# XinkeAE/Active-ORB-SLAM2

Hardware: AMD Instinct MI355X
Metric: frames/sec (extract+match+localBA) TUM 640x480 (higher is better)
Workload: dtype u8 (extract, match) + f64 (PoseOptimization, LocalBA)

## Files before the change

active-orb-slam2_amd/capi.py:

```python
from __future__ import annotations

import ctypes as C
import os

import numpy as np

_HERE = os.path.dirname(os.path.abspath(__file__))
_LIB = None

AOS2_OK = 0
AOS2_ERR_ARG, AOS2_ERR_CAPACITY, AOS2_ERR_TOO_SMALL, AOS2_ERR_HIP, AOS2_ERR_NO_DEVICE = -1, -2, -3, -4, -5
AOS2_ERR_STOPPED = 1

KP_DTYPE = np.dtype([("x", "<f4"), ("y", "<f4"), ("size", "<f4"), ("angle", "<f4"),
                     ("response", "<f4"), ("octave", "<i4"), ("class_id", "<i4")])


class LibraryMissing(RuntimeError):
    pass


class AosError(RuntimeError):
    def __init__(self, code, msg):
        super().__init__(f"aos2 error {code}: {msg}")
# ... 23 lines not shown
        for n in ("scale_factors", "inv_scale_factors", "sigma2", "inv_sigma2"):
            f = getattr(L, "aos2_extractor_" + n)
            f.argtypes = [vp]
            f.restype = C.POINTER(cf)
        for n in ("features_per_level", "umax"):
            f = getattr(L, "aos2_extractor_" + n)
            f.argtypes = [vp]
            f.restype = C.POINTER(ci)
        L.aos2_extractor_max_keypoints.argtypes = [vp]
        L.aos2_extractor_max_keypoints_for.argtypes = [vp, ci, ci]
        L.aos2_extractor_extract.argtypes = [vp, vp, ci, ci, ci, vp, vp, ci, C.POINTER(ci)]
        L.aos2_extractor_extract_batch.argtypes = [vp, vp, ci, ci, ci, ci, C.c_size_t, vp, vp, ci, vp]
        L.aos2_host_alloc.argtypes = [C.POINTER(vp), C.c_size_t]
        L.aos2_host_free.argtypes = [vp]
        L.aos2_extractor_extract_batch_device.argtypes = [vp, vp, ci, ci, ci, ci, C.c_size_t, vp, vp, ci, vp]
        L.aos2_extractor_extract_batch_device_async.argtypes = [vp, vp, ci, ci, ci, ci, C.c_size_t, vp, vp, ci, vp]
        L.aos2_extractor_wait.argtypes = [vp]
        L.aos2_extractor_pyramid_level_size.argtypes = [vp, ci, C.POINTER(ci), C.POINTER(ci)]
        L.aos2_extractor_pyramid_level.argtypes = [vp, ci, ci, ci, vp, ci]
        L.aos2_extractor_debug_candidates.argtypes = [vp, ci, ci, vp, vp, vp, ci, C.POINTER(ci)]
        L.aos2_extractor_last_timing.argtypes = [vp, vp, ci]
        if hasattr(L, "aos2_extractor_set_chunks"):
            L.aos2_extractor_set_chunks.argtypes = [vp, ci]
        L.aos2_extractor_bench_fast.argtypes = [vp, ci, C.POINTER(cf)]
        L.aos2_extractor_bench_describe.argtypes = [vp, ci, C.POINTER(cf)]
        if hasattr(L, "aos2_compute_stereo_matches"):
            L.aos2_compute_stereo_matches.argtypes = [vp, vp, ci, vp, vp, ci, vp, vp, ci, cf, cf, vp, vp]
            L.aos2_compute_stereo_matches_device.argtypes = [vp, vp, ci, vp, vp, vp, vp, vp, vp, ci, cf, cf, vp, vp]
            L.aos2_compute_stereo_matches_device_async.argtypes = [vp, vp, ci, vp, vp, vp, vp, vp, vp, ci, cf, cf, vp, vp]
            L.aos2_compute_stereo_matches_last_device_ms.restype = cf
            L.aos2_compute_stereo_matches_last_device_ms.argtypes = [vp]
        if hasattr(L, "aos2_vocabulary_create"):
            L.aos2_vocabulary_create.argtypes = [ci, C.POINTER(vp)]
            L.aos2_vocabulary_destroy.argtypes = [vp]
            L.aos2_vocabulary_load_binary.argtypes = [vp, C.c_char_p]
            L.aos2_vocabulary_load_text.argtypes = [vp, C.c_char_p]
            L.aos2_vocabulary_save_binary.argtypes = [vp, C.c_char_p]
            L.aos2_vocabulary_set_nodes.argtypes = [vp, ci, ci, ci, ci, ci, vp, vp, vp, vp]
            for nm in ("k", "levels", "scoring", "weighting", "nodes", "empty"):
                getattr(L, "aos2_vocabulary_" + nm).argtypes = [vp]
            L.aos2_vocabulary_size.argtypes = [vp]
            L.aos2_vocabulary_get_nodes.argtypes = [vp] * 6
            L.aos2_vocabulary_size.restype = C.c_uint
            L.aos2_vocabulary_transform.argtypes = [vp, vp, ci, ci, vp, vp, C.POINTER(ci), vp, vp, vp, C.POINTER(ci), vp, vp]
            L.aos2_vocabulary_transform_device.argtypes = [vp, ci, vp, vp, ci, ci] + [vp] * 9
            L.aos2_vocabulary_last_device_ms.restype = cf
            L.aos2_vocabulary_last_device_ms.argtypes = [vp]
            L.aos2_vocabulary_score.argtypes = [vp, vp, vp, ci, vp, vp, ci, C.POINTER(C.c_double)]
        L.aos2_debug_octree_host.argtypes = [vp, vp, vp, ci, ci, ci, ci, ci, ci, vp, ci]
        L.aos2_debug_sincos_host.argtypes = [cf, C.POINTER(cf), C.POINTER(cf)]
        L.aos2_debug_extractor_plan.argtypes = [vp, ci, ci, vp, vp, ci, C.POINTER(ci), vp]
        L.aos2_debug_sincos_device.argtypes = [vp, ci, vp, vp, ci]
        L.aos2_debug_wave_ops_device.argtypes = [vp, vp, ci, ci, vp, vp, ci]
        L.aos2_debug_pose_blocks_device.argtypes = [vp, vp, vp, vp, vp, vp, vp, ci, ci]
        L.aos2_debug_lba_reduced_solve_device.argtypes = [ci] + [vp] * 12 + [ci]
        L.aos2_debug_triangulate_host.argtypes = [vp, ci, vp, vp, vp, vp]
        L.aos2_triangulate_matches.argtypes = [vp, vp, ci, vp, vp, vp, vp]
        L.aos2_debug_sim3_host.argtypes = [vp, vp, ci]
        L.aos2_sim3_ransac.argtypes = [vp, vp, vp, ci]
        L.aos2_debug_pnp_host.argtypes = [vp, vp, ci]
        L.aos2_debug_pnp_set.argtypes = [ci, vp, ci, vp]
        L.aos2_debug_pnp_scan.argtypes = [ci, ci, vp, vp, ci, ci, ci, vp, vp, vp]
        L.aos2_pnp_ransac.argtypes = [vp, vp, vp, ci]
        L.aos2_pnp_ransac_parameters.argtypes = [ci, C.c_double, ci, ci, ci, cf, vp, vp, vp]
        L.aos2_debug_sim3_opt_host.argtypes = [vp, vp, ci]
        L.aos2_optimize_sim3.argtypes = [vp, vp, vp, ci]
        L.aos2_optimize_sim3_last_device_ms.argtypes = [vp]
        L.aos2_optimize_sim3_last_device_ms.restype = cf
        if hasattr(L, "aos2_matcher_create"):
            L.aos2_matcher_create.argtypes = [cf, ci, ci, C.POINTER(vp)]
            L.aos2_matcher_destroy.argtypes = [vp]
            L.aos2_descriptor_distance.argtypes = [vp, vp]
            if hasattr(L, "aos2_matcher_last_device_ms"):
                L.aos2_matcher_last_device_ms.argtypes = [vp]
                L.aos2_matcher_last_device_ms.restype = cf
            L.aos2_matcher_hamming_best2.argtypes = [vp, vp, ci, vp, ci, vp, vp, vp]
            L.aos2_matcher_hamming_best2_device.argtypes = [vp, vp, ci, vp, ci, vp, vp, vp, ci, C.POINTER(cf)]
            L.aos2_matcher_search_by_bow.argtypes = [vp, vp, ci, vp, vp]
            L.aos2_matcher_search_by_bow_device.argtypes = [vp, vp, ci, vp, vp]
            L.aos2_matcher_search_by_bow_frames.argtypes = [vp, vp, vp, vp]
            L.aos2_vocabulary_stream.argtypes = [vp]
            L.aos2_vocabulary_stream.restype = vp
            if hasattr(L, "aos2_matcher_search_by_bow_kf"):
                L.aos2_matcher_search_by_bow_kf.argtypes = [vp, vp, ci, vp, vp]
                L.aos2_matcher_search_for_triangulation.argtypes = [vp, vp, ci, ci, vp, vp]
                L.aos2_compute_distinctive_descriptors.argtypes = [vp, ci, vp, vp, vp]
            if hasattr(L, "aos2_matcher_fuse"):
                L.aos2_matcher_fuse.argtypes = [vp, vp, vp, ci, vp, vp, vp]
                L.aos2_matcher_search_by_projection_kf.argtypes = [vp, vp, vp, vp, vp]
                L.aos2_matcher_search_by_sim3.argtypes = [vp, vp, vp, vp, vp, vp, vp]
                L.aos2_matcher_search_by_projection_reloc.argtypes = [vp, vp, vp, ci, vp, vp]
            if hasattr(L, "aos2_frame_assign_features_to_grid"):
                L.aos2_frame_assign_features_to_grid.argtypes = [vp, ci, vp, vp, cf, cf, cf, cf, vp, vp, C.POINTER(C.c_int32)]
                L.aos2_frame_stereo_from_rgbd.argtypes = [vp, ci, vp, vp, vp, vp, ci, ci, ci, cf, vp, vp]
            if hasattr(L, "aos2_frame_is_in_frustum"):
                L.aos2_frame_is_in_frustum.argtypes = [vp, vp, cf, cf, cf, cf, ci, cf, vp, vp, vp, vp, vp, vp]
            if hasattr(L, "aos2_matcher_search_for_initialization"):
                L.aos2_matcher_search_for_initialization.argtypes = [vp, vp, ci, vp, vp, vp, vp, ci, vp, vp]
            if hasattr(L, "aos2_matcher_search_by_projection_batch"):
                L.aos2_matcher_search_by_projection_batch.argtypes = [vp, vp, vp, ci, cf, vp, vp]
            L.aos2_matcher_search_by_projection.argtypes = [vp, vp, vp, cf, vp, vp]
            L.aos2_matcher_search_by_projection_last.argtypes = [vp, vp, vp, cf, ci, vp, vp]
        if hasattr(L, "aos2_lba_create"):
            L.aos2_lba_create.argtypes = [ci, C.POINTER(vp)]
            L.aos2_lba_destroy.argtypes = [vp]
            L.aos2_lba_solve.argtypes = [vp, vp, vp]
# ... 833 lines not shown
        for k, a in zip(names, arr):
            setattr(P[i], k, a.ctypes.data)
        for tag, K in (("1", q["K1"]), ("2", q["K2"])):
            for name, v in zip(("fx", "fy", "cx", "cy"), K):
                setattr(P[i], name + tag, float(np.float32(v)))
        P[i].q12 = (C.c_double * 4)(*[float(v) for v in q["q12"]])
        P[i].t12 = (C.c_double * 3)(*[float(v) for v in q["t12"]])
        P[i].s12, P[i].th2, P[i].fix_scale = float(q["s12"]), float(np.float32(q["th2"])), int(bool(q["fix_scale"]))
        R[i].outlier = out.ctypes.data
        if sentinel is not None:
            C.memset(C.byref(R[i]), sentinel, _Sim3OptResult.outlier.offset)
            R[i].n_bad = R[i].n_inliers = sentinel
    return P, R, keep, outs


def _sim3_opt_results(R, outs):
    return [dict(q12=np.array(R[i].q12, np.float64), t12=np.array(R[i].t12, np.float64), s12=np.float64(R[i].s12), outlier=out,
                 n_bad=R[i].n_bad, n_inliers=R[i].n_inliers, iterations=tuple(R[i].iterations), trials=tuple(R[i].trials))
            for i, out in enumerate(outs)]


def debug_sim3_opt_host(problems):
    P, R, keep, outs = _sim3_opt_args(problems)
    _check(lib().aos2_debug_sim3_opt_host(P, R, len(problems)))
    return _sim3_opt_results(R, outs)


def debug_sincos_device(angles, device=0):
    a = np.ascontiguousarray(angles, np.float32)
    s = np.zeros_like(a)
    c = np.zeros_like(a)
    _check(lib().aos2_debug_sincos_device(_p(a), len(a), _p(s), _p(c), device))
    return s, c


WAVE_OPS_I = ("dpp_u32_B1", "dpp_u32_4E", "dpp_u32_141", "dpp_u32_140", "dpp_i32_B1", "dpp_i32_4E", "dpp_i32_141", "dpp_i32_140",
              "row_sum", "sum", "max", "row_min", "min", "incl_scan", "block_excl_scan", "block_total")
WAVE_OPS_D = ("dpp_f64_B1", "dpp_f64_4E", "dpp_f64_141", "dpp_f64_140", "row_sum_f64", "readlane_0", "readlane_63")


def debug_wave_ops_device(vi, vd, device=0):
    vi = np.ascontiguousarray(vi, np.int32); vd = np.ascontiguousarray(vd, np.float64)
    assert vi.ndim == 2 and vi.shape == vd.shape
    oi = np.zeros(vi.shape + (len(WAVE_OPS_I),), np.int32)
    od = np.zeros(vi.shape + (len(WAVE_OPS_D),), np.float64)
    _check(lib().aos2_debug_wave_ops_device(_p(vi), _p(vd), vi.shape[0], vi.shape[1], _p(oi), _p(od), device))
    out = {k: oi[..., j].copy() for j, k in enumerate(WAVE_OPS_I)}
    out.update({k: od[..., j].copy() for j, k in enumerate(WAVE_OPS_D)})
    for k in ("row_min", "min"):
        out[k] = out[k].view(np.uint32)
    return out


def debug_pose_blocks_device(upd, T, Hb, lam, x0, device=0):
    upd = np.ascontiguousarray(upd, np.float64); T = np.ascontiguousarray(T, np.float64)
    Hb = np.ascontiguousarray(Hb, np.float64); lam = np.ascontiguousarray(lam, np.float64)
    x = np.ascontiguousarray(x0, np.float64).copy()
    n = len(lam)
    To = np.zeros((n, 7)); ok = np.zeros(n, np.uint8)
    _check(lib().aos2_debug_pose_blocks_device(_p(upd), _p(T), _p(To), _p(Hb), _p(lam), _p(x), _p(ok), n, device))
    return To, x, ok


def debug_lba_reduced_solve_device(cases, device=0):
    cat = lambda k, dt=np.float64: np.ascontiguousarray(np.concatenate([np.asarray(c[k], dt).ravel() for c in cases]))
    nps = np.array([np.asarray(c["bs"]).size // 6 for c in cases], np.int32)
    for c, q in zip(cases, nps):
        assert np.asarray(c["H"]).shape == (6 * q, 6 * q) and np.asarray(c["T"]).shape == (q, 7)
        assert all(np.asarray(c[k]).shape == (6 * q,) for k in ("bs", "b_pose", "x0", "scale0"))
    form = np.array([c["form"] for c in cases], np.int32)
    H, bs, bp, T, x, sc = cat("H"), cat("bs"), cat("b_pose"), cat("T"), cat("x0"), cat("scale0")
    lam = np.array([c["lam"] for c in cases], np.float64)
    To, Tb, ok = np.zeros_like(T), np.zeros_like(T), np.zeros(len(cases), np.uint8)
    _check(lib().aos2_debug_lba_reduced_solve_device(len(cases), _p(nps), _p(form), _p(H), _p(bs), _p(bp), _p(lam), _p(T), _p(x), _p(To), _p(Tb),
                                                     _p(sc), _p(ok), device))
    out, o6, o7 = [], 0, 0
    for q, k in zip(nps, ok):
        out.append(dict(ok=int(k), x=x[o6:o6 + 6 * q].copy(), scale_terms=sc[o6:o6 + 6 * q].copy(),
                        T_out=To[o7:o7 + 7 * q].reshape(q, 7).copy(), T_backup=Tb[o7:o7 + 7 * q].reshape(q, 7).copy()))
        o6 += 6 * q; o7 += 7 * q
    return out


class _BowPair(C.Structure):
    _fields_ = [("n_kf", C.c_int32), ("n_f", C.c_int32), ("desc_kf", C.c_void_p), ("desc_f", C.c_void_p),
                ("kf_has_mp", C.c_void_p), ("angle_kf", C.c_void_p), ("angle_f", C.c_void_p),
                ("n_nodes_kf", C.c_int32), ("n_nodes_f", C.c_int32),
                ("node_id_kf", C.c_void_p), ("node_off_kf", C.c_void_p), ("node_idx_kf", C.c_void_p),
                ("node_id_f", C.c_void_p), ("node_off_f", C.c_void_p), ("node_idx_f", C.c_void_p)]


class _BowFrames(C.Structure):
    _fields_ = [("n_frames", C.c_int32), ("cap", C.c_int32)] + [(k, C.c_void_p) for k in (
        "d_desc_kf", "d_kps_kf", "d_n_kf", "d_desc_f", "d_kps_f", "d_n_f", "kf_has_mp", "d_kf_fv_node", "d_kf_fv_off", "d_kf_fv_idx",
        "d_kf_n_fv", "d_f_fv_node", "d_f_fv_off", "d_f_fv_idx", "d_f_n_fv")]


class _BowKfPair(C.Structure):
    _fields_ = [("n1", C.c_int32), ("n2", C.c_int32), ("desc1", C.c_void_p), ("desc2", C.c_void_p),
                ("has_mp1", C.c_void_p), ("has_mp2", C.c_void_p), ("angle1", C.c_void_p), ("angle2", C.c_void_p),
                ("n_nodes1", C.c_int32), ("n_nodes2", C.c_int32),
                ("node_id1", C.c_void_p), ("node_off1", C.c_void_p), ("node_idx1", C.c_void_p),
                ("node_id2", C.c_void_p), ("node_off2", C.c_void_p), ("node_idx2", C.c_void_p)]


class _TriangPair(C.Structure):
# ... 663 lines not shown
```

active-orb-slam2_amd/csrc/debug_taps.hip:

```cpp
#include <algorithm>
#include <cmath>
#include <vector>

#include "aos2_common.h"
#include "octree.h"
#include "pnp.h"
#include "sincos_exact.h"
#include "sim3.h"
#include "triangulate.h"
#include "wave_ops.h"

namespace aos2 {
__global__ void sincos_kernel(const float *a, int n, float *s, float *c)
{
    const int i = blockIdx.x * blockDim.x + threadIdx.x;
    if (i < n) sincos_exact(a[i], &s[i], &c[i]);
}

constexpr int kWaveOpsI = 16, kWaveOpsD = 7;
template <int NT>
__global__ __launch_bounds__(NT) void wave_ops_kernel(const int32_t *vi, const double *vd, int32_t *out_i, double *out_d)
{
    __shared__ int32_t wsum[NT / 64];
    const size_t t = (size_t)blockIdx.x * NT + threadIdx.x;
    const int v = vi[t];
    const double d = vd[t];
    int32_t *oi = out_i + kWaveOpsI * t;
    double *od = out_d + kWaveOpsD * t;
    oi[0] = (int32_t)dpp_u32<0xB1>((uint32_t)v);
    oi[1] = (int32_t)dpp_u32<0x4E>((uint32_t)v);
    oi[2] = (int32_t)dpp_u32<0x141>((uint32_t)v);
    oi[3] = (int32_t)dpp_u32<0x140>((uint32_t)v);
    oi[4] = dpp_i32<0xB1>(v);
    oi[5] = dpp_i32<0x4E>(v);
    oi[6] = dpp_i32<0x141>(v);
    oi[7] = dpp_i32<0x140>(v);
    oi[8] = wave_row_sum_i32(v);
    oi[9] = wave_sum_i32(v);
    oi[10] = wave_max_i32(v);
    oi[11] = (int32_t)wave_row_min_u32((uint32_t)v);
    oi[12] = (int32_t)wave_min_u32((uint32_t)v);
    oi[13] = wave_incl_scan_i32(v);
    int total;
    oi[14] = block_excl_scan_i32<NT>(v, wsum, total);
    oi[15] = total;
    od[0] = dpp_f64<0xB1>(d);
    od[1] = dpp_f64<0x4E>(d);
    od[2] = dpp_f64<0x141>(d);
    od[3] = dpp_f64<0x140>(d);
    od[4] = row_sum_f64(d);
    od[5] = readlane_f64(d, 0);
    od[6] = readlane_f64(d, 63);
}

int triang_check(const aos2_triang_geom_t *g, int n, const aos2_triang_obs_t *obs1, const aos2_triang_obs_t *obs2, const float *x3D,
                 const uint8_t *status)
{
    if (!g || n < 0 || (n > 0 && (!obs1 || !obs2 || !x3D || !status)) || g->n_levels < 2 || g->n_levels > 8) {
        set_error("bad argument (geometry, per-match arrays, 2..8 pyramid levels)");
        return AOS2_ERR_ARG;
    }
    for (int k = 0; k < n; ++k)
        if (obs1[k].octave < 0 || obs1[k].octave >= g->n_levels || obs2[k].octave < 0 || obs2[k].octave >= g->n_levels) {
            set_error("match %d: octaves (%d, %d) outside the %d pyramid levels", k, obs1[k].octave, obs2[k].octave, g->n_levels);
            return AOS2_ERR_ARG;
        }
    return AOS2_OK;
}

static int32_t sim3_ransac_its(int n, double probability, int min_inliers, int max_iterations)
{
    const float epsilon = (float)min_inliers / n;
    int nIterations;
    if (min_inliers == n) nIterations = 1;
    else {
        const double v = ceil(log(1 - probability) / log(1 - pow((double)epsilon, 3)));
        nIterations = (v >= -2147483648.0 && v <= 2147483647.0) ? (int)v : INT32_MIN;
    }
    return std::max(1, std::min(nIterations, max_iterations));
}

int sim3_check(const aos2_sim3_problem_t *problems, const aos2_sim3_result_t *results, int n_problems, int32_t *its, uint8_t *run)
{
    if (n_problems < 0 || n_problems > 64 || (n_problems > 0 && (!problems || !results))) {
        set_error("bad argument (0..64 problems and their results)");
        return AOS2_ERR_ARG;
    }
    for (int p = 0; p < n_problems; ++p) {
        const aos2_sim3_problem_t &P = problems[p];
        if (P.n < 0 || P.max_iterations < 1 || (P.n > 0 && (!P.X3Dc1 || !P.X3Dc2 || !P.max_err1 || !P.max_err2 || !results[p].inliers))) {
            set_error("problem %d: bad argument (n >= 0, max_iterations >= 1, the per-correspondence arrays)", p);
            return AOS2_ERR_ARG;
        }
        its[p] = sim3_ransac_its(P.n, P.probability, P.min_inliers, P.max_iterations);
        run[p] = P.n >= P.min_inliers;
        if (!run[p]) continue;
        if (P.n < 3 || !P.draws) {
            set_error("problem %d: %d correspondences to draw triples from, or no draws", p, P.n);
            return AOS2_ERR_ARG;
        }
        for (int k = 0; k < P.max_iterations; ++k)
            for (int i = 0; i < 3; ++i) {
                const int32_t r = P.draws[3 * (size_t)k + i];
                if (r < 0 || r > P.n - 1 - i) {
                    set_error("problem %d: draw %d of iteration %d is %d, outside [0, %d]", p, i, k, r, P.n - 1 - i);
                    return AOS2_ERR_ARG;
                }
// ... 241 lines not shown
                           int minY, int maxY, int N, int32_t *out_idx, int cap)
{
    using namespace aos2;
    if (n <= 0) return 0;
    const int mn = oct_max_nodes(n, N);
    std::vector<OctNode> nodes(mn);
    std::vector<int32_t> perm(n), tmp(n), pairs((size_t)4 * mn);
    OctScratch S{nodes.data(), perm.data(), tmp.data(), pairs.data(), pairs.data() + 2 * mn, mn, mn};
    return distribute_octree(xs, ys, score, n, minX, maxX, minY, maxY, N, S, out_idx, cap);
}

void aos2_debug_sincos_host(float angle_rad, float *s, float *c) { aos2::sincos_exact(angle_rad, s, c); }

int aos2_debug_sincos_device(const float *angles, int n, float *s, float *c, int device)
{
    using namespace aos2;
    int st;
    if ((st = bind_device(device))) return st;
    DevBuf<float> da, ds, dc;
    if ((st = da.alloc(n)) || (st = ds.alloc(n)) || (st = dc.alloc(n))) return st;
    AOS2_HIP_CHECK(hipMemcpy(da.p, angles, sizeof(float) * n, hipMemcpyHostToDevice));
    hipLaunchKernelGGL(sincos_kernel, dim3((n + 255) / 256), dim3(256), 0, 0, da.p, n, ds.p, dc.p);
    AOS2_HIP_CHECK(hipDeviceSynchronize());
    AOS2_HIP_CHECK(hipMemcpy(s, ds.p, sizeof(float) * n, hipMemcpyDeviceToHost));
    AOS2_HIP_CHECK(hipMemcpy(c, dc.p, sizeof(float) * n, hipMemcpyDeviceToHost));
    da.release(); ds.release(); dc.release();
    return AOS2_OK;
}

int aos2_debug_wave_ops_device(const int32_t *vi, const double *vd, int n_cases, int nt, int32_t *out_i, double *out_d, int device)
{
    using namespace aos2;
    if (!vi || !vd || !out_i || !out_d || n_cases < 1 || (nt != 128 && nt != 256)) {
        set_error("bad argument (the four arrays, >= 1 cases, 128 or 256 threads: the sizes the library scans with)");
        return AOS2_ERR_ARG;
    }
    int st;
    if ((st = bind_device(device))) return st;
    const size_t n = (size_t)n_cases * nt;
    DevBuf<int32_t> di, doi;
    DevBuf<double> dd, dod;
    if ((st = di.alloc(n)) || (st = dd.alloc(n)) || (st = doi.alloc(kWaveOpsI * n)) || (st = dod.alloc(kWaveOpsD * n))) return st;
    AOS2_HIP_CHECK(hipMemcpy(di.p, vi, sizeof(int32_t) * n, hipMemcpyHostToDevice));
    AOS2_HIP_CHECK(hipMemcpy(dd.p, vd, sizeof(double) * n, hipMemcpyHostToDevice));
    if (nt == 128) hipLaunchKernelGGL(wave_ops_kernel<128>, dim3(n_cases), dim3(128), 0, 0, di.p, dd.p, doi.p, dod.p);
    else hipLaunchKernelGGL(wave_ops_kernel<256>, dim3(n_cases), dim3(256), 0, 0, di.p, dd.p, doi.p, dod.p);
    AOS2_HIP_CHECK(hipDeviceSynchronize());
    AOS2_HIP_CHECK(hipMemcpy(out_i, doi.p, sizeof(int32_t) * kWaveOpsI * n, hipMemcpyDeviceToHost));
    AOS2_HIP_CHECK(hipMemcpy(out_d, dod.p, sizeof(double) * kWaveOpsD * n, hipMemcpyDeviceToHost));
    di.release(); dd.release(); doi.release(); dod.release();
    return AOS2_OK;
}

int aos2_png_unfilter(uint8_t *rows, int h, int stride, int bpp)
{
    if (!rows || h < 0 || stride <= 0 || bpp <= 0) return AOS2_ERR_ARG;
    const size_t pitch = (size_t)stride + 1;
    for (int y = 0; y < h; ++y) {
        uint8_t *cur = rows + (size_t)y * pitch + 1;
        const uint8_t *up = y ? rows + (size_t)(y - 1) * pitch + 1 : nullptr;
        const int ft = rows[(size_t)y * pitch];
        for (int x = 0; x < stride; ++x) {
            const int a = x >= bpp ? cur[x - bpp] : 0, b = up ? up[x] : 0, c = (up && x >= bpp) ? up[x - bpp] : 0;
            int pred = 0;
            switch (ft) {
            case 0: break;
            case 1: pred = a; break;
            case 2: pred = b; break;
            case 3: pred = (a + b) >> 1; break;
            case 4: {
                const int p = a + b - c, pa = abs(p - a), pb = abs(p - b), pc = abs(p - c);
                pred = (pa <= pb && pa <= pc) ? a : (pb <= pc ? b : c);
                break;
            }
            default: return AOS2_ERR_ARG;
            }
            cur[x] = (uint8_t)(cur[x] + pred);
        }
    }
    return AOS2_OK;
}

}
```

active-orb-slam2_amd/csrc/lba.hip:

```cpp
#include <dlfcn.h>

#include <chrono>
#include <cstdio>
#include <cstdlib>
#include <memory>
#include <numeric>
#include <atomic>
#include <condition_variable>
#include <functional>
#include <mutex>
#include <thread>

#include "lba_math.h"
#include "ldlt_reg.h"
#include "wave_ops.h"

namespace aos2 {

struct Cam {
    double fx, fy, cx, cy, bf;
    float bf_f;
    double delta_mono, delta_stereo;
};

// ... 722 lines not shown
    double H[9] = {0, 0, 0, 0, 0, 0, 0, 0, 0}, bl[3] = {0, 0, 0};
    const int e0 = W.pt_off[l], e1 = W.pt_off[l + 1];
    for (int a = e0; a < e1; a += kWalkChunkLin) {
        int kk[kWalkChunkLin], ep[kWalkChunkLin], ph[kWalkChunkLin];
        uint8_t lv1[kWalkChunkLin], ste[kWalkChunkLin], rob[kWalkChunkLin];
        double T[kWalkChunkLin][7], er[kWalkChunkLin][3], ew[kWalkChunkLin];
#pragma unroll
        for (int u = 0; u < kWalkChunkLin; ++u) kk[u] = W.pt_k[min(a + u, e1 - 1)];
#pragma unroll
        for (int u = 0; u < kWalkChunkLin; ++u) {
            ep[u] = W.e_pose[kk[u]];
            ph[u] = W.pl_pos[kk[u]];
            lv1[u] = W.e_level1[kk[u]];
            ste[u] = W.e_stereo[kk[u]];
            rob[u] = W.e_robust[kk[u]];
            ew[u] = (double)W.in_w[kk[u]];
#pragma unroll
            for (int i = 0; i < 3; ++i) er[u][i] = (double)W.in_obs[3 * (size_t)kk[u] + i];
        }
#pragma unroll
        for (int u = 0; u < kWalkChunkLin; ++u)
#pragma unroll
            for (int i = 0; i < 7; ++i) T[u][i] = W.pose[7 * (size_t)ep[u] + i];
#pragma unroll
        for (int u = 0; u < kWalkChunkLin; ++u) {
            if (a + u >= e1) break;
            if (lv1[u]) continue;
            const int stereo = ste[u];
            double p[3], R[9];
            se3_map(T[u], Xv, p);
            rot_from_quat(T[u], R);
            double Ja[9];
            jac_point(W.cam, R, p, stereo, Ja);
            double omr[3], wo;
            double res[3];
            edge_error(W.cam, p, er[u], stereo, res);
            edge_weights_of(W.cam, res, ew[u], rob[u], stereo, omr, wo);
#pragma unroll
            for (int r = 0; r < 3; ++r) {
                bl[r] += Ja[r] * omr[0] + Ja[3 + r] * omr[1] + Ja[6 + r] * omr[2];
#pragma unroll
                for (int c = 0; c < 3; ++c) H[r * 3 + c] += Ja[r] * wo * Ja[c] + Ja[3 + r] * wo * Ja[3 + c] + Ja[6 + r] * wo * Ja[6 + c];
            }
            if (ph[u] >= 0) lrec_store(W, ph[u], p, wo, stereo, omr);
        }
    }
    for (int i = 0; i < 9; ++i) W.Hll[9 * (size_t)l + i] = H[i];
    for (int i = 0; i < 3; ++i) W.b[6 * (size_t)W.np + 3 * (size_t)l + i] = bl[i];
}

template <int K, int NT = 256>
__device__ __forceinline__ double workgroup_sum_k256(double (&acc)[K], double *red , int n_items)
{
    const int lane = threadIdx.x & 63, row = threadIdx.x >> 4, wave = threadIdx.x >> 6;
    const int rows_used = min(NT / 16, (n_items + 15) >> 4);
    if (wave * 64 < n_items) {
#pragma unroll
        for (int i = 0; i < K; ++i) acc[i] = row_sum_f64(acc[i]);
        if ((lane & 15) == 0) {
#pragma unroll
            for (int i = 0; i < K; ++i) red[row * (K + 1) + i] = acc[i];
        }
    }
    __syncthreads();
    double sum = 0;
    if ((int)threadIdx.x < K)
        for (int r = 0; r < rows_used; ++r) sum += red[r * (K + 1) + threadIdx.x];
    return sum;
}

__device__ __forceinline__ void lin_poses_body(const LbaWin &W, int ph, int init)
{
    __shared__ double red[16 * 43];
    if (ph >= W.np) return;
    double T[7];
    {
        const double *Tp = W.pose + 7 * (size_t)W.hpose[ph];
#pragma unroll
        for (int i = 0; i < 7; ++i) T[i] = Tp[i];
    }
    if (threadIdx.x == 0) {
        double R[9];
        rot_from_quat(T, R);
#pragma unroll
        for (int i = 0; i < 9; ++i) W.Rl[9 * (size_t)ph + i] = R[i];
    }
    if (!init) return;
    double acc[42];
#pragma unroll
    for (int i = 0; i < 42; ++i) acc[i] = 0;
    for (int a = W.ps_off[ph] + threadIdx.x; a < W.ps_off[ph + 1]; a += 256) {
        const int k = W.ps_k[a];
        if (W.e_level1[k]) continue;
        const int stereo = W.e_stereo[k];
        double p[3], Jb[18], omr[3], wo;
        se3_map(T, W.point + 3 * (size_t)W.e_point[k], p);
        jac_pose(W.cam, p, stereo, Jb);
        edge_weights(W, k, p, stereo, omr, wo);
#pragma unroll
        for (int r = 0; r < 6; ++r) {
            acc[36 + r] += Jb[r] * omr[0] + Jb[6 + r] * omr[1] + Jb[12 + r] * omr[2];
#pragma unroll
            for (int c = 0; c < 6; ++c) acc[r * 6 + c] += Jb[r] * wo * Jb[c] + Jb[6 + r] * wo * Jb[6 + c] + Jb[12 + r] * wo * Jb[12 + c];
        }
    }
    const double sum = workgroup_sum_k256<42>(acc, red, W.ps_off[ph + 1] - W.ps_off[ph]);
    if (threadIdx.x < 36)
        W.Hpp[36 * (size_t)ph + threadIdx.x] = sum;
    else if (threadIdx.x < 42)
        W.b[6 * (size_t)ph + (threadIdx.x - 36)] = sum;
}

template <bool kWalk>
__global__ __launch_bounds__(256) __attribute__((amdgpu_waves_per_eu(3, 3))) void k_lin(const LbaWin *__restrict__ wins, const SchurTask *__restrict__ tasks, int init)
{
// ... 138 lines not shown
        if (!kDiag || c >= 5) acc[30 + c] += -(La.iz * u[2]);
    }
    if (kDiag) {
        const double o[3] = {W.lomr[3 * (size_t)kb], W.lomr[3 * (size_t)kb + 1], W.lomr[3 * (size_t)kb + 2]};
        double bp[6] = {0, 0, 0, 0, 0, 0};
        lrec_bp(W.cam, ra, o, bp);
        acc[6] += bp[0]; acc[12] += bp[1]; acc[13] += bp[2]; acc[18] += bp[3]; acc[19] += bp[4]; acc[20] += bp[5];
    }
}

__device__ __forceinline__ void schur_store(const LbaWin &W, int i1, int i2, int e, double sum, double lambda)
{
    const bool diag = i1 == i2;
    if (e < 36) {
        double v = -sum;
        const int r = e / 6, c = e - 6 * r;
        if (diag && r == c) v += lambda;
        W.Hs[(size_t)(6 * i1 + r) * W.hs_ld + 6 * i2 + c] = v;
        if (!diag) W.Hs[(size_t)(6 * i2 + c) * W.hs_ld + 6 * i1 + r] = v;
    }
}

__global__ __launch_bounds__(kSchurThreads) __attribute__((amdgpu_waves_per_eu(3, 3)))
void k_schur(const LbaWin *__restrict__ wins, const SchurTask *__restrict__ tasks)
{
    constexpr int NT = kSchurThreads;
    __shared__ double red[(NT / 16) * 43];
    __shared__ int32_t s_info[16], s_ij[16];
    const SchurTask tk = tasks[blockIdx.x];
    if (tk.w < 0) return;
    const LbaWin &W = wins[tk.w];
    const int run = W.st->run;
    const double lambda = W.st->lambda;
    const int np = W.np, n6 = 6 * np;
    const int kind = tk.code >> 28, arg = tk.code & 0x0fffffff;
    const int tid = threadIdx.x, lane = tid & 63, wave = tid >> 6;
    double acc[42];
#pragma unroll
    for (int i = 0; i < 42; ++i) acc[i] = 0;
    if (kind == kSchurPack) {
        const int row = tid >> 4, li = tid & 15, r = arg + row;
        int o0 = 0, info = 0, ij = 0;
        if (r < W.n_srows) {
            o0 = W.sr_o0[r];
            info = W.sr_info[r];
            ij = W.sr_ij[r];
        }
        if (!run) return;
        if (li == 0) {
            s_info[row] = info;
            s_ij[row] = ij;
        }
        if (li < (info & 255)) schur_item<false>(W, o0 + li, lambda, n6, W.Rl + 9 * (size_t)(ij & 0xffff), W.Rl + 9 * (size_t)(ij >> 16), acc);
#pragma unroll
        for (int i = 0; i < 36; ++i) acc[i] = row_sum_f64(acc[i]);
        if (li == 0) {
#pragma unroll
            for (int i = 0; i < 36; ++i) red[row * 43 + i] = acc[i];
        }
        __syncthreads();
        for (int rr = wave; rr < 16; rr += NT / 64) {
            const int inf = s_info[rr], nrb = (inf >> 16) & 255;
            if (((inf >> 8) & 255) != 0 || nrb == 0 || lane >= 36) continue;
            double sum = 0;
            for (int k = 0; k < nrb; ++k) sum += red[(rr + k) * 43 + lane];
            schur_store(W, s_ij[rr] & 0xffff, s_ij[rr] >> 16, lane, sum, lambda);
        }
        return;
    }
    int i1, i2;
    if (kind == kSchurDiag)
        i1 = i2 = arg;
    else {
        int rem = arg;
        i1 = 0;
        while (rem >= np - i1) {
            rem -= np - i1;
            ++i1;
        }
        i2 = i1 + rem;
    }
    const int blk = i1 * np - i1 * (i1 - 1) / 2 + (i2 - i1);
    const int o0 = W.blk_off[blk], n = W.blk_off[blk + 1] - o0;
    if (!run) return;
    if (kind == kSchurDiag)
        for (int j = tid; j < n; j += NT) schur_item<true>(W, o0 + j, lambda, n6, W.Rl + 9 * (size_t)i1, W.Rl + 9 * (size_t)i1, acc);
    else
        for (int j = tid; j < n; j += NT) schur_item<false>(W, o0 + j, lambda, n6, W.Rl + 9 * (size_t)i1, W.Rl + 9 * (size_t)i2, acc);
    const double sum = workgroup_sum_k256<42, NT>(acc, red, n);
    if (kind != kSchurDiag) {
        schur_store(W, i1, i2, tid, sum, lambda);
        return;
    }
    __shared__ double s_bsum[6];
    if (tid >= 36 && tid < 42) s_bsum[tid - 36] = sum;
    __syncthreads();
    if (tid < 36) {
        const int r = tid / 6, c = tid - 6 * r;
        if (r <= c) {
            double v = -sum;
            if (r == c) v += lambda;
            W.Hs[(size_t)(6 * i1 + r) * W.hs_ld + 6 * i1 + c] = v;
            if (r != c) W.Hs[(size_t)(6 * i1 + c) * W.hs_ld + 6 * i1 + r] = v;
        } else {
            const int j = tid == 6 ? 0 : tid == 12 ? 1 : tid == 13 ? 2 : tid == 18 ? 3 : tid == 19 ? 4 : tid == 20 ? 5 : -1;
            if (j >= 0) {
                W.b[6 * i1 + j] = sum;
                W.bs[6 * i1 + j] = sum - s_bsum[j];
            }
        }
    }
}
// ... 1747 lines not shown
```

active-orb-slam2_amd/csrc/wave_ops.h:

```cpp
#pragma once
#include <hip/hip_runtime.h>

namespace aos2 {

template <int kCtrl>
__device__ __forceinline__ uint32_t dpp_u32(uint32_t v)
{
    return (uint32_t)__builtin_amdgcn_update_dpp((int)v, (int)v, kCtrl, 0xf, 0xf, false);
}
template <int kCtrl>
__device__ __forceinline__ int dpp_i32(int v)
{
    return __builtin_amdgcn_update_dpp(0, v, kCtrl, 0xf, 0xf, false);
}
template <int kCtrl>
__device__ __forceinline__ double dpp_f64(double v)
{
    const long long b = __double_as_longlong(v);
    const int lo = __builtin_amdgcn_update_dpp((int)b, (int)b, kCtrl, 0xf, 0xf, false);
    const int hi = __builtin_amdgcn_update_dpp((int)(b >> 32), (int)(b >> 32), kCtrl, 0xf, 0xf, false);
    return __longlong_as_double(((long long)hi << 32) | (unsigned int)lo);
}

__device__ __forceinline__ double readlane_f64(double v, int src)
{
    const long long bits = __double_as_longlong(v);
    const int lo = __builtin_amdgcn_readlane((int)(bits & 0xffffffffll), src);
    const int hi = __builtin_amdgcn_readlane((int)(bits >> 32), src);
    return __longlong_as_double(((long long)hi << 32) | (unsigned int)lo);
}

__device__ __forceinline__ int wave_row_sum_i32(int v)
{
    v += dpp_i32<0xB1>(v);
    v += dpp_i32<0x4E>(v);
    v += dpp_i32<0x141>(v);
    v += dpp_i32<0x140>(v);
    return v;
}

__device__ __forceinline__ int wave_sum_i32(int v)
{
    v = wave_row_sum_i32(v);
    return __builtin_amdgcn_readlane(v, 0) + __builtin_amdgcn_readlane(v, 16) + __builtin_amdgcn_readlane(v, 32) +
           __builtin_amdgcn_readlane(v, 48);
}

__device__ __forceinline__ int wave_max_i32(int v)
{
    v = max(v, dpp_i32<0xB1>(v));
    v = max(v, dpp_i32<0x4E>(v));
    v = max(v, dpp_i32<0x141>(v));
    v = max(v, dpp_i32<0x140>(v));
    return max(max(__builtin_amdgcn_readlane(v, 0), __builtin_amdgcn_readlane(v, 16)),
               max(__builtin_amdgcn_readlane(v, 32), __builtin_amdgcn_readlane(v, 48)));
}

__device__ __forceinline__ uint32_t wave_row_min_u32(uint32_t k)
{
    k = min(k, dpp_u32<0xB1>(k));
    k = min(k, dpp_u32<0x4E>(k));
    k = min(k, dpp_u32<0x141>(k));
    k = min(k, dpp_u32<0x140>(k));
    return k;
}

__device__ __forceinline__ uint32_t wave_min_u32(uint32_t k)
{
    k = wave_row_min_u32(k);
    uint32_t a = __builtin_amdgcn_readlane(k, 0);
    a = min(a, (uint32_t)__builtin_amdgcn_readlane(k, 16));
    a = min(a, (uint32_t)__builtin_amdgcn_readlane(k, 32));
    a = min(a, (uint32_t)__builtin_amdgcn_readlane(k, 48));
    return a;
}

__device__ __forceinline__ double row_sum_f64(double v)
{
    v += dpp_f64<0xB1>(v);
    v += dpp_f64<0x4E>(v);
    v += dpp_f64<0x141>(v);
    v += dpp_f64<0x140>(v);
    return v;
}

__device__ __forceinline__ int wave_incl_scan_i32(int v)
{
    int x = v;
    x += __builtin_amdgcn_update_dpp(0, x, 0x111, 0xf, 0xf, false);
    x += __builtin_amdgcn_update_dpp(0, x, 0x112, 0xf, 0xf, false);
    x += __builtin_amdgcn_update_dpp(0, x, 0x114, 0xf, 0xf, false);
    x += __builtin_amdgcn_update_dpp(0, x, 0x118, 0xf, 0xf, false);
    x += __builtin_amdgcn_update_dpp(0, x, 0x142, 0xa, 0xf, false);
    x += __builtin_amdgcn_update_dpp(0, x, 0x143, 0xc, 0xf, false);
    return x;
}

template <int NT>
__device__ __forceinline__ int block_excl_scan_i32(int v, int32_t *wsum, int &total)
{
    static_assert(NT % 64 == 0, "whole waves");
    const int lane = threadIdx.x & 63, wave = threadIdx.x >> 6;
    const int incl = wave_incl_scan_i32(v);
    if (lane == 63) wsum[wave] = incl;
    __syncthreads();
    int excl = incl - v;
    total = 0;
#pragma unroll
    for (int w = 0; w < NT / 64; ++w) {
        if (w == wave) excl += total;
        total += wsum[w];
    }
    return excl;
}

}
```

include/aos2.h:

```cpp
#ifndef AOS2_H
#define AOS2_H

#include <stddef.h>
#include <stdint.h>

#ifdef __cplusplus
extern "C" {
#endif

#define AOS2_OK 0
#define AOS2_ERR_ARG (-1)
#define AOS2_ERR_CAPACITY (-2)
#define AOS2_ERR_TOO_SMALL (-3)
#define AOS2_ERR_HIP (-4)
#define AOS2_ERR_NO_DEVICE (-5)
#define AOS2_ERR_STOPPED (1)

const char *aos2_last_error(void);
int aos2_device_count(void);
const char *aos2_version(void);
int aos2_device_local_cpus(int device, char *buf, int cap);


typedef struct {
// ... 503 lines not shown
                                         int32_t *d_nmatches);
int aos2_frames_fuse(aos2_frames_t *kfs, const aos2_map_points_dev_t *mps, int n_problems, int n_pts,
                     const int32_t *target, const int32_t *d_rows, float th, int32_t *d_best_idx,
                     int32_t *d_best_dist);
int aos2_frames_set_async_keyframe_calls(aos2_frames_t *f, int on);

#define AOS2_TRI_NO_MATCH 0
#define AOS2_TRI_ACCEPTED 1
#define AOS2_TRI_LOW_PARALLAX 2
#define AOS2_TRI_W_ZERO 3
#define AOS2_TRI_DEPTH1 4
#define AOS2_TRI_DEPTH2 5
#define AOS2_TRI_REPROJ1 6
#define AOS2_TRI_REPROJ2 7
#define AOS2_TRI_ZERO_DIST 8
#define AOS2_TRI_SCALE 9
#define AOS2_TRI_SUPERSEDED 10
int aos2_frames_triangulate_matches(aos2_frames_t *a, aos2_frames_t *b, int n_pairs, const int32_t *kf1, const int32_t *kf2,
                                    const int32_t *d_match12, int first_wins, float *d_x3D, uint8_t *d_status,
                                    int32_t *d_nnew);
typedef struct {
    float Tcw1[16], Tcw2[16];
    float fx1, fy1, cx1, cy1, mb1, mbf1;
    float fx2, fy2, cx2, cy2, mb2, mbf2;
    int32_t n_levels;
    float scale_factors1[8], scale_factors2[8];
} aos2_triang_geom_t;
typedef struct {
    float ux, uy;
    float kx, ky;
    float u_right;
    float depth;
    int32_t octave;
} aos2_triang_obs_t;
int aos2_triangulate_matches(aos2_matcher_t *m, const aos2_triang_geom_t *g, int n, const aos2_triang_obs_t *obs1,
                             const aos2_triang_obs_t *obs2, float *x3D, uint8_t *status);

typedef struct aos2_graph aos2_graph_t;
int aos2_capture_begin(void *hip_stream);
int aos2_capture_end(void *hip_stream, aos2_graph_t **out);
int aos2_graph_launch(aos2_graph_t *g, void *hip_stream);
int aos2_graph_nodes(const aos2_graph_t *g);
void aos2_graph_destroy(aos2_graph_t *g);

int aos2_png_unfilter(uint8_t *rows, int h, int stride, int bpp);

int aos2_debug_octree_host(const int16_t *xs, const int16_t *ys, const uint8_t *score, int n,
                           int minX, int maxX, int minY, int maxY, int N, int32_t *out_idx, int cap);
int aos2_debug_extractor_plan(const aos2_extractor_t *e, int w, int h, int64_t *levels, int32_t *cells, int cell_cap,
                              int *n_cells, int64_t *totals);
void aos2_debug_sincos_host(float angle_rad, float *s, float *c);
int aos2_debug_sincos_device(const float *angles, int n, float *s, float *c, int device);
int aos2_debug_wave_ops_device(const int32_t *vi, const double *vd, int n_cases, int nt, int32_t *out_i, double *out_d, int device);
int aos2_debug_triangulate_host(const aos2_triang_geom_t *g, int n, const aos2_triang_obs_t *obs1,
                                const aos2_triang_obs_t *obs2, float *x3D, uint8_t *status);
int aos2_debug_sim3_host(const aos2_sim3_problem_t *problems, aos2_sim3_result_t *results, int n_problems);
int aos2_debug_pnp_host(const aos2_pnp_problem_t *problems, aos2_pnp_result_t *results, int n_problems);
int aos2_debug_pnp_set(int n, const int32_t *row, int min_set, int32_t *indices);
int aos2_debug_pnp_scan(int first_iteration, int n_iterations, const int32_t *counts, const int32_t *refined, int32_t refined_carried,
                        int min_inliers, int best_inliers_in, int32_t *returned_at, int32_t *best_iteration, int32_t *best_inliers);
int aos2_debug_sim3_opt_host(const aos2_sim3_opt_problem_t *p, aos2_sim3_opt_result_t *r, int n_problems);
int aos2_debug_pose_blocks_device(const double *upd, const double *T, double *T_out, const double *Hb, const double *lambda,
                                  double *x, uint8_t *ok, int n, int device);
int aos2_debug_lba_reduced_solve_device(int n_cases, const int32_t *np, const int32_t *form, const double *H, const double *bs,
                                        const double *b_pose, const double *lambda, const double *T, double *x, double *T_out,
                                        double *T_backup, double *scale_terms, uint8_t *ok, int device);

typedef struct {
    int32_t np, nl, npad;
    int32_t phase;
    int32_t trials_first, iters_done_first;
    int32_t n_units;
    double lambda, current_chi;
    int32_t *hpose, *hpoint;
    int32_t *blk_off;
    int32_t *units;
    double *pose, *point;
    uint8_t *e_level1, *e_robust;
    double *Hpp_init, *b_init;
    double *b_p;
    double *Hll, *b_l;
    double *Hs, *bs;
} aos2_lba_system_t;
int aos2_debug_lba_assemble_device(aos2_lba_t *s, const aos2_lba_problem_t *problems, int n_problems, int layout, int stage,
                                   const double *lambda, aos2_lba_system_t *out);

#ifdef __cplusplus
}
#endif
#endif
```

Baseline: 74430.

## Replace per-value row sums with recursive-halving scatter reduction in LBA workgroup sums

```diff
diff --git a/active-orb-slam2_amd/capi.py b/active-orb-slam2_amd/capi.py
--- a/active-orb-slam2_amd/capi.py
+++ b/active-orb-slam2_amd/capi.py
@@ -99,6 +99,7 @@
         L.aos2_debug_extractor_plan.argtypes = [vp, ci, ci, vp, vp, ci, C.POINTER(ci), vp]
         L.aos2_debug_sincos_device.argtypes = [vp, ci, vp, vp, ci]
         L.aos2_debug_wave_ops_device.argtypes = [vp, vp, ci, ci, vp, vp, ci]
+        L.aos2_debug_row_sums_scatter_device.argtypes = [vp, ci, vp, vp, ci]
         L.aos2_debug_pose_blocks_device.argtypes = [vp, vp, vp, vp, vp, vp, vp, ci, ci]
         L.aos2_debug_lba_reduced_solve_device.argtypes = [ci] + [vp] * 12 + [ci]
         L.aos2_debug_triangulate_host.argtypes = [vp, ci, vp, vp, vp, vp]
@@ -1038,6 +1039,16 @@
     return out
 
 
+def debug_row_sums_scatter_device(v, device=0):
+    v = np.ascontiguousarray(v, np.float64)
+    assert v.ndim == 2 and v.shape[0] == 64
+    K = v.shape[1]
+    out = np.zeros((64, (K + 15) // 16), np.float64)
+    owner = np.zeros((K, 2), np.int32)
+    _check(lib().aos2_debug_row_sums_scatter_device(_p(v), K, _p(out), _p(owner), device))
+    return out, owner
+
+
 def debug_pose_blocks_device(upd, T, Hb, lam, x0, device=0):
     upd = np.ascontiguousarray(upd, np.float64); T = np.ascontiguousarray(T, np.float64)
     Hb = np.ascontiguousarray(Hb, np.float64); lam = np.ascontiguousarray(lam, np.float64)
diff --git a/active-orb-slam2_amd/csrc/debug_taps.hip b/active-orb-slam2_amd/csrc/debug_taps.hip
--- a/active-orb-slam2_amd/csrc/debug_taps.hip
+++ b/active-orb-slam2_amd/csrc/debug_taps.hip
@@ -53,6 +53,38 @@
     od[6] = readlane_f64(d, 63);
 }
 
+template <int K>
+__global__ __launch_bounds__(64) void row_sums_scatter_kernel(const double *v, double *out)
+{
+    double a[K];
+#pragma unroll
+    for (int i = 0; i < K; ++i) a[i] = v[K * threadIdx.x + i];
+    row_sums_scatter_f64<K>(a);
+#pragma unroll
+    for (int s = 0; s < row_scatter_slots(K); ++s) out[row_scatter_slots(K) * threadIdx.x + s] = a[s];
+}
+
+template <int K>
+int row_sums_scatter_run(const double *v, double *out, int32_t *owner)
+{
+    constexpr int S = row_scatter_slots(K);
+    int st;
+    DevBuf<double> dv, dout;
+    if ((st = dv.alloc(64 * K)) || (st = dout.alloc(64 * S))) return st;
+    AOS2_HIP_CHECK(hipMemcpy(dv.p, v, sizeof(double) * 64 * K, hipMemcpyHostToDevice));
+    hipLaunchKernelGGL(row_sums_scatter_kernel<K>, dim3(1), dim3(64), 0, 0, dv.p, dout.p);
+    AOS2_HIP_CHECK(hipDeviceSynchronize());
+    AOS2_HIP_CHECK(hipMemcpy(out, dout.p, sizeof(double) * 64 * S, hipMemcpyDeviceToHost));
+    dv.release(); dout.release();
+    for (int i = 0; i < K; ++i) {
+        int li = 0, s = 0;
+        row_scatter_owner<K>(i, li, s);
+        owner[2 * i] = li;
+        owner[2 * i + 1] = s;
+    }
+    return AOS2_OK;
+}
+
 int triang_check(const aos2_triang_geom_t *g, int n, const aos2_triang_obs_t *obs1, const aos2_triang_obs_t *obs2, const float *x3D,
                  const uint8_t *status)
 {
@@ -400,6 +432,17 @@
     return AOS2_OK;
 }
 
+int aos2_debug_row_sums_scatter_device(const double *v, int K, double *out, int32_t *owner, int device)
+{
+    using namespace aos2;
+    if (!v || !out || !owner || (K != 7 && K != 36 && K != 42)) {
+        set_error("bad argument (the three arrays, K = 7, 36 or 42)");
+        return AOS2_ERR_ARG;
+    }
+    if (int st = bind_device(device)) return st;
+    return K == 7 ? row_sums_scatter_run<7>(v, out, owner) : K == 36 ? row_sums_scatter_run<36>(v, out, owner) : row_sums_scatter_run<42>(v, out, owner);
+}
+
 int aos2_png_unfilter(uint8_t *rows, int h, int stride, int bpp)
 {
     if (!rows || h < 0 || stride <= 0 || bpp <= 0) return AOS2_ERR_ARG;
diff --git a/active-orb-slam2_amd/csrc/lba.hip b/active-orb-slam2_amd/csrc/lba.hip
--- a/active-orb-slam2_amd/csrc/lba.hip
+++ b/active-orb-slam2_amd/csrc/lba.hip
@@ -798,15 +798,11 @@
 template <int K, int NT = 256>
 __device__ __forceinline__ double workgroup_sum_k256(double (&acc)[K], double *red , int n_items)
 {
-    const int lane = threadIdx.x & 63, row = threadIdx.x >> 4, wave = threadIdx.x >> 6;
+    const int row = threadIdx.x >> 4, wave = threadIdx.x >> 6;
     const int rows_used = min(NT / 16, (n_items + 15) >> 4);
     if (wave * 64 < n_items) {
-#pragma unroll
-        for (int i = 0; i < K; ++i) acc[i] = row_sum_f64(acc[i]);
-        if ((lane & 15) == 0) {
-#pragma unroll
-            for (int i = 0; i < K; ++i) red[row * (K + 1) + i] = acc[i];
-        }
+        row_sums_scatter_f64<K>(acc);
+        row_scatter_store<K>(acc, red + row * (K + 1));
     }
     __syncthreads();
     double sum = 0;
@@ -1051,12 +1047,8 @@
             s_ij[row] = ij;
         }
         if (li < (info & 255)) schur_item<false>(W, o0 + li, lambda, n6, W.Rl + 9 * (size_t)(ij & 0xffff), W.Rl + 9 * (size_t)(ij >> 16), acc);
-#pragma unroll
-        for (int i = 0; i < 36; ++i) acc[i] = row_sum_f64(acc[i]);
-        if (li == 0) {
-#pragma unroll
-            for (int i = 0; i < 36; ++i) red[row * 43 + i] = acc[i];
-        }
+        row_sums_scatter_f64<36>(acc);
+        row_scatter_store<36>(acc, red + row * 43);
         __syncthreads();
         for (int rr = wave; rr < 16; rr += NT / 64) {
             const int inf = s_info[rr], nrb = (inf >> 16) & 255;
diff --git a/active-orb-slam2_amd/csrc/wave_ops.h b/active-orb-slam2_amd/csrc/wave_ops.h
--- a/active-orb-slam2_amd/csrc/wave_ops.h
+++ b/active-orb-slam2_amd/csrc/wave_ops.h
@@ -17,8 +17,16 @@
 __device__ __forceinline__ double dpp_f64(double v)
 {
     const long long b = __double_as_longlong(v);
-    const int lo = __builtin_amdgcn_update_dpp((int)b, (int)b, kCtrl, 0xf, 0xf, false);
-    const int hi = __builtin_amdgcn_update_dpp((int)(b >> 32), (int)(b >> 32), kCtrl, 0xf, 0xf, false);
+    const int lo = __builtin_amdgcn_update_dpp(0, (int)b, kCtrl, 0xf, 0xf, true);
+    const int hi = __builtin_amdgcn_update_dpp(0, (int)(b >> 32), kCtrl, 0xf, 0xf, true);
+    return __longlong_as_double(((long long)hi << 32) | (unsigned int)lo);
+}
+template <int kCtrl, int kBanks>
+__device__ __forceinline__ double dpp_f64_banks(double old, double v)
+{
+    const long long o = __double_as_longlong(old), b = __double_as_longlong(v);
+    const int lo = __builtin_amdgcn_update_dpp((int)o, (int)b, kCtrl, 0xf, kBanks, false);
+    const int hi = __builtin_amdgcn_update_dpp((int)(o >> 32), (int)(b >> 32), kCtrl, 0xf, kBanks, false);
     return __longlong_as_double(((long long)hi << 32) | (unsigned int)lo);
 }
 
@@ -84,6 +92,74 @@
     return v;
 }
 
+constexpr int row_scatter_count(int K, int level) { return level == 0 ? K : ((K + (1 << level) - 1) >> level); }
+constexpr int row_scatter_slots(int K) { return row_scatter_count(K, 4); }
+template <int K>
+__host__ __device__ constexpr int row_scatter_index(int s, int li)
+{
+    constexpr int n0 = K, n1 = row_scatter_count(K, 1), n2 = row_scatter_count(K, 2), n3 = row_scatter_count(K, 3);
+    int idx = s;
+    idx = ((n3 & 1) && idx == n3 / 2) ? n3 - 1 : 2 * idx + ((li >> 3) & 1);
+    idx = ((n2 & 1) && idx == n2 / 2) ? n2 - 1 : 2 * idx + ((li >> 2) & 1);
+    idx = ((n1 & 1) && idx == n1 / 2) ? n1 - 1 : 2 * idx + ((li >> 1) & 1);
+    idx = ((n0 & 1) && idx == n0 / 2) ? n0 - 1 : 2 * idx + (li & 1);
+    return idx;
+}
+template <int K>
+__host__ __device__ constexpr void row_scatter_owner(int i, int &li, int &s)
+{
+    for (li = 0; li < 16; ++li)
+        for (s = 0; s < row_scatter_slots(K); ++s)
+            if (row_scatter_index<K>(s, li) == i) return;
+}
+
+template <int kCtrl>
+__device__ __forceinline__ double row_scatter_pair_quad(double a, double b, bool up)
+{
+    const double keep = up ? b : a, send = up ? a : b;
+    return keep + dpp_f64<kCtrl>(send);
+}
+template <int kFromUp, int kFromLo, int kLo>
+__device__ __forceinline__ double row_scatter_pair_banks(double a, double b)
+{
+    const double x = dpp_f64_banks<kFromLo, 0xf & ~kLo>(a, b);
+    const double y = dpp_f64_banks<kFromUp, kLo>(b, a);
+    return x + y;
+}
+__device__ __forceinline__ double row_scatter_single_4(double v)
+{
+    return v + dpp_f64_banks<0x114, 0xa>(dpp_f64_banks<0x104, 0x5>(v, v), v);
+}
+
+template <int K, int N>
+__device__ __forceinline__ void row_sums_scatter_f64(double (&v)[N])
+{
+    static_assert(K >= 1 && K <= N, "K values of the array");
+    const int lane = threadIdx.x & 15;
+    constexpr int n0 = K, n1 = row_scatter_count(K, 1), n2 = row_scatter_count(K, 2), n3 = row_scatter_count(K, 3);
+    const bool up0 = lane & 1, up1 = lane & 2;
+#pragma unroll
+    for (int m = 0; m < n0 / 2; ++m) v[m] = row_scatter_pair_quad<0xB1>(v[2 * m], v[2 * m + 1], up0);
+    if (n0 & 1) v[n0 / 2] = v[n0 - 1] + dpp_f64<0xB1>(v[n0 - 1]);
+#pragma unroll
+    for (int m = 0; m < n1 / 2; ++m) v[m] = row_scatter_pair_quad<0x4E>(v[2 * m], v[2 * m + 1], up1);
+    if (n1 & 1) v[n1 / 2] = v[n1 - 1] + dpp_f64<0x4E>(v[n1 - 1]);
+#pragma unroll
+    for (int m = 0; m < n2 / 2; ++m) v[m] = row_scatter_pair_banks<0x104, 0x114, 0x5>(v[2 * m], v[2 * m + 1]);
+    if (n2 & 1) v[n2 / 2] = row_scatter_single_4(v[n2 - 1]);
+#pragma unroll
+    for (int m = 0; m < n3 / 2; ++m) v[m] = row_scatter_pair_banks<0x128, 0x128, 0x3>(v[2 * m], v[2 * m + 1]);
+    if (n3 & 1) v[n3 / 2] = v[n3 - 1] + dpp_f64<0x128>(v[n3 - 1]);
+}
+template <int K, int N, int S = 0>
+__device__ __forceinline__ void row_scatter_store(const double (&v)[N], double *out)
+{
+    if constexpr (S < row_scatter_slots(K)) {
+        out[row_scatter_index<K>(S, threadIdx.x & 15)] = v[S];
+        row_scatter_store<K, N, S + 1>(v, out);
+    }
+}
+
 __device__ __forceinline__ int wave_incl_scan_i32(int v)
 {
     int x = v;
diff --git a/include/aos2.h b/include/aos2.h
--- a/include/aos2.h
+++ b/include/aos2.h
@@ -579,6 +579,7 @@
 void aos2_debug_sincos_host(float angle_rad, float *s, float *c);
 int aos2_debug_sincos_device(const float *angles, int n, float *s, float *c, int device);
 int aos2_debug_wave_ops_device(const int32_t *vi, const double *vd, int n_cases, int nt, int32_t *out_i, double *out_d, int device);
+int aos2_debug_row_sums_scatter_device(const double *v, int K, double *out, int32_t *owner, int device);
 int aos2_debug_triangulate_host(const aos2_triang_geom_t *g, int n, const aos2_triang_obs_t *obs1,
                                 const aos2_triang_obs_t *obs2, float *x3D, uint8_t *status);
 int aos2_debug_sim3_host(const aos2_sim3_problem_t *problems, aos2_sim3_result_t *results, int n_problems);
```

After: 76380 (median of 6 runs). 2.6% higher.
